# xuyongzhi/Automatic-As-built-Reconstruction

Measured on AMD Instinct MI355X. Metric: scenes/sec (fwd+bwd), higher is better.
Workload: dtype f32

## Files before the change

automatic-as-built-reconstruction_amd/_hip.py:

```python
import ctypes as C
import os

import torch

_HERE = os.path.dirname(os.path.abspath(__file__))
LIB_PATH = os.path.join(_HERE, "lib", "libaabr_hip.so")

_lib = None
META_WORDS = 16
ABI_VERSION = 640

_vp, _i64, _i32, _f32 = C.c_void_p, C.c_int64, C.c_int, C.c_float
_i32p = C.POINTER(C.c_int32)
_f32p = C.POINTER(C.c_float)
_i64p = C.POINTER(C.c_int64)



class AabrRoiLevel(C.Structure):
    _fields_ = [("feats", C.c_void_p), ("cellmap", C.c_void_p), ("height", C.c_int32), ("width", C.c_int32),
                ("zsize", C.c_int32), ("nb", C.c_int32), ("V", C.c_int64), ("row_offset", C.c_int64),
                ("spatial_scale", C.c_float), ("reserved", C.c_int32)]


class AabrRpnMap(C.Structure):
    _fields_ = [("features", C.c_void_p), ("rows", C.c_int64), ("objectness", C.c_void_p),
                ("box_regression", C.c_void_p), ("d_features", C.c_void_p)]


class AabrMlpWindow(C.Structure):
    _fields_ = [("n_rois", C.c_int64), ("ph", C.c_int32), ("pw", C.c_int32), ("R", C.c_int32), ("wlen", C.c_int32),
                ("blocks", C.c_int32), ("w0", C.c_int32 * 2)]


_lvp = C.POINTER(AabrRoiLevel)
_mwp = C.POINTER(AabrMlpWindow)
_rmp = C.POINTER(AabrRpnMap)
_ppv = C.POINTER(C.c_void_p)
_SIGS = {
    "aabr_version": (C.c_int, []),
    "aabr_build_flags": (C.c_int, []),
    "aabr_last_error": (C.c_char_p, []),
    "aabr_set_knob": (C.c_int, [C.c_char_p, C.c_int, C.c_int]),
    "aabr_quantize_points": (C.c_int, [_vp, _i32, _i64, C.c_double, _vp, _vp, _i64, _vp, _vp, _i32, _vp]),
    "aabr_input_layer_status_words": (C.c_int64, [_i64]),
    "aabr_input_layer_sites": (C.c_int, [_vp, _i64, _i32, _vp, _i64, _vp, _vp, _vp, _vp, _vp, _vp, _vp, _vp, _vp, _vp]),
    "aabr_input_layer_pack_bits": (C.c_int, [_i64, _i32p]),
# ... 74 lines not shown
    "aabr_bn_backward_parts": (C.c_int, [_vp, _vp, _vp, _vp, _i64, _i32, _vp, _vp, _vp, _vp, _vp, _vp, _f32, _vp, _i32,
                                         _vp, _vp, _vp]),
    "aabr_bn_forward_parts": (C.c_int, [_vp, _vp, _i64, _i32, _vp, _vp, _vp, _vp, _vp, _vp, _f32, _f32, _f32, _vp,
                                        _i32, _vp, _vp]),
    "aabr_bn_forward_parts_bf16": (C.c_int, [_vp, _vp, _i64, _i32, _vp, _vp, _vp, _vp, _vp, _vp, _f32, _f32, _f32, _vp,
                                             _i32, _vp, _vp]),
    "aabr_mailbox_create": (C.c_int, [_i64, _vp]),
    "aabr_mailbox_destroy": (C.c_int, [_vp]),
    "aabr_mailbox_post": (C.c_int, [_vp, _i64, _vp, C.c_uint32, _vp]),
    "aabr_conv_wpack_floats": (C.c_int64, [_i32, _i32, _i32]),
    "aabr_conv_forward": (C.c_int, [_vp, _i32, _i64, _vp, _i32, _i64, _vp, _i32, _vp, _vp, _i32, _vp, _vp]),
    "aabr_conv_dw_scratch_floats": (C.c_int64, [_i64, _i32, _i32]),
    "aabr_conv_backward_weight": (C.c_int, [_vp, _i32, _vp, _i32, _i64, _vp, _i32, _i64, _vp, _vp, _vp, _vp]),
    "aabr_conv_dw_chunk_pairs": (C.c_int, [_i64, _i32, _i32, _i32]),
    "aabr_conv_dw_vec_operands": (C.c_int, [_i32, _vp, _i32, _vp, _i32, _i64, _i32, _i64]),
    "aabr_conv_pack_weights2": (C.c_int, [_vp, _i32, _i32, _i32, _vp, _vp, _vp]),
    "aabr_conv_pack_weights2_bf16": (C.c_int, [_vp, _i32, _i32, _i32, _vp, _vp, _vp]),
    "aabr_plan_run": (C.c_int, [_vp, _i32, _vp]),
    "aabr_plan_run_tail": (C.c_int, [_vp, _i32, _vp, C.POINTER(C.c_uint64)]),
    "aabr_plan_tail_join": (C.c_int, [C.c_uint64, _vp]),
    "aabr_plan_tail_sync": (C.c_int, [C.c_uint64]),
    "aabr_plan_tail_release": (C.c_int, [C.c_uint64]),
    "aabr_plan_submit": (C.c_int, [_vp, _i32, _vp, _i32]),
    "aabr_plan_drain": (C.c_int, []),
    "aabr_plan_launcher_stats": (None, [_vp, _vp, _vp]),
    "aabr_geom_run": (C.c_int, [_vp, _i32, _vp]),
    "aabr_add": (C.c_int, [_vp, _vp, _vp, _i64, _i32, _vp]),
    "aabr_cast_storage": (C.c_int, [_vp, _vp, _i64, _i32, _vp]),
    "aabr_sum_counts": (C.c_int, [_vp, _vp, _vp, _i32, _vp]),
    "aabr_conv_pack_job_blocks": (C.c_int64, [_i32, _i32, _i32]),
# ... 346 lines not shown
```

automatic-as-built-reconstruction_amd/csrc/common.h:

```cpp
#pragma once
#include <hip/hip_runtime.h>
#include <stdint.h>
#include <stdio.h>
#include <atomic>
#include "../../include/aabr_hip.h"
#include "conv_tiles.h"

namespace aabr {

void set_error(const char *fmt, ...);

typedef float f32x4 __attribute__((ext_vector_type(4)));
typedef unsigned int u32x4 __attribute__((ext_vector_type(4)));
typedef __bf16 bf16x8 __attribute__((ext_vector_type(8)));

#define AABR_KNOB_LIST(X)                                                                                            \
  X(CONV_WLDS) X(CONV_SMALL) X(CONV_NBW) X(CONV_WPB) X(WIDE_ROWS) X(CONV_WIDE) X(WIDE_NBUF) X(CONV_WIDE_BF16)         \
  X(VOXEL_MEAN) X(WIDE_NCB) X(BN_SMALL) X(WIDE_PRIO) X(PLAN_SIDE_BATCH) X(PLAN_SIDE_PRIO) X(SMALL_WPB) X(SMALL_MAX)   \
  X(WIDE_SPLIT) X(SPLIT_TARGET) X(SPLIT_NBUF) X(SPLIT_MIN_ITEMS) X(CONV_NARROW) X(DW_FULL) X(DW_FULL_MIN) X(DW_FULL_WGS) X(DW_VEC) X(SPLIT_ROWS) X(GEOM_JOBS)      \
  X(CONV_SINGLE) X(SINGLE_ROWS) X(SINGLE_CHUNK) X(SINGLE_BWD_STATS) X(PLAN_TAIL)
#define AABR_KNOB_ENUM(n) K_##n,
enum Knob { AABR_KNOB_LIST(AABR_KNOB_ENUM) K_COUNT };
#undef AABR_KNOB_ENUM
int knob(Knob k);

#define AABR_CHECK_ARG_AS(fn, cond, msg)                            \
  do {                                                              \
    if (!(cond)) { aabr::set_error("%s: %s", fn, msg); return AABR_EINVAL; } \
  } while (0)
#define AABR_CHECK_ARG(cond, msg) AABR_CHECK_ARG_AS(__func__, cond, msg)

#define AABR_CHECK_LAUNCH()                                                   \
  do {                                                                        \
    hipError_t e__ = hipGetLastError();                                       \
    if (e__ != hipSuccess) {                                                  \
// ... 110 lines not shown
```

automatic-as-built-reconstruction_amd/csrc/conv_dw.hip:

```cpp
#include "common.h"
#include "conv_dw_tiles.h"
#include "offset_pairs.h"

namespace aabr {

extern thread_local const char *g_last_variant;

__device__ inline float ldf(const float *p, int64_t i) { return p[i]; }
__device__ inline float ldf(const __bf16 *p, int64_t i) { return (float)p[i]; }

typedef float f32x2 __attribute__((ext_vector_type(2)));
template <int N> __device__ inline void ld_row(float (&d)[N], const float *p) {
  if constexpr (N == 4) {
    const f32x4 v = *reinterpret_cast<const f32x4 *>(p);
    d[0] = v[0]; d[1] = v[1]; d[2] = v[2]; d[3] = v[3];
  } else if constexpr (N == 2) {
    const f32x2 v = *reinterpret_cast<const f32x2 *>(p);
    d[0] = v[0]; d[1] = v[1];
  } else d[0] = p[0];
}
template <int N> __device__ inline void ld_row(__bf16 (&)[N], const __bf16 *) {}
template <bool V> struct DwForm { static constexpr bool value = V; };

template <int CB, int NB, typename T>
__global__ __launch_bounds__(256) __attribute__((amdgpu_waves_per_eu(2))) void k_conv_dw_pairs(const T *__restrict__ in, int ci,
                                                       const T *__restrict__ d_out, int co, int64_t V,
                                                       const int32_t *__restrict__ words, int vol,
                                                       int chunk_pairs, float *__restrict__ partial, int form) {
  __shared__ f32x4 red[CB * NB][64];
  constexpr bool kF32 = sizeof(T) == 4;
  const int direct = form & 1;
  const bool vin = kF32 && CB > 1 && (form & (kDwVecIn << 1)), vout = kF32 && NB > 1 && (form & (kDwVecOut << 1));
  const int wave = threadIdx.x >> 6, lane = threadIdx.x & 63;
  const int g = lane >> 4, c16 = lane & 15;
  const int nnb = nnb_of(co);
  const int tiles_n = (nnb + NB - 1) / NB;
  const int tile = blockIdx.y;
  const int cb0 = (tile / tiles_n) * CB, nb0 = (tile % tiles_n) * NB;
  const int chunk = blockIdx.x;
  int k, c0, c1;
  if (!dw_chunk_range(words, vol, chunk_pairs, direct, chunk, lane, k, c0, c1)) return;
  const int rk = words[k];
  const int p0 = c0 + wave * (chunk_pairs / 4);
  int p1 = p0 + chunk_pairs / 4;
  if (p1 > c1) p1 = c1;
  const int2 *pairs = reinterpret_cast<const int2 *>(words + op_hdr(vol) + (int64_t)vol * op_nb256(V)) +
                      (int64_t)k * V;
  f32x4 acc[CB][NB];
#pragma unroll
  for (int a = 0; a < CB; ++a)
#pragma unroll
    for (int b = 0; b < NB; ++b) acc[a][b] = (f32x4){0.f, 0.f, 0.f, 0.f};

  const int cA = ci - 1, nA = co - 1;
// ... 118 lines not shown
    }
  }
#pragma unroll
  for (int a = 0; a < CB; ++a)
#pragma unroll
    for (int b = 0; b < NB; ++b) {
      f32x4 t = red[a * NB + b][lane];
#pragma unroll
      for (int r = 0; r < 4; ++r) {
        int c = cb0 * 16 + dw_tile_row(vin, CB, g, r, a), n = nb0 * 16 + dw_tile_col(vout, NB, c16, b);
        if (c < ci && n < co) P[(int64_t)c * co + n] = t[r];
      }
    }
}

typedef short s16x4 __attribute__((ext_vector_type(4)));

template <int CB, int NB>
__global__ __launch_bounds__(256) void k_conv_dw_pairs_bf16(const __bf16 *__restrict__ in, int ci,
                                                            const __bf16 *__restrict__ d_out, int co, int64_t V,
                                                            const int32_t *__restrict__ words, int vol,
                                                            int chunk_pairs, float *__restrict__ partial, int direct) {
  constexpr int SX = CB * 32 + 16, SG = NB * 32 + 16;
  constexpr int XCH = CB * 2, GCH = NB * 2;
  constexpr int XIT = (32 * XCH) / 64, GIT = (32 * GCH) / 64;
  __shared__ f32x4 red[CB * NB][64];
  __shared__ __attribute__((aligned(16))) unsigned char stage[4][32 * (SX + SG)];
  const int wave = threadIdx.x >> 6, lane = threadIdx.x & 63;
  const int g = lane >> 4, c16 = lane & 15;
  const int nnb = nnb_of(co);
  const int tiles_n = (nnb + NB - 1) / NB;
  const int tile = blockIdx.y;
  const int cb0 = (tile / tiles_n) * CB, nb0 = (tile % tiles_n) * NB;
  const int chunk = blockIdx.x;
  int k, c0, c1;
  if (!dw_chunk_range(words, vol, chunk_pairs, direct, chunk, lane, k, c0, c1)) return;
  const int p0 = c0 + wave * (chunk_pairs / 4);
  int p1 = p0 + chunk_pairs / 4;
  if (p1 > c1) p1 = c1;
  const int2 *pairs = reinterpret_cast<const int2 *>(words + op_hdr(vol) + (int64_t)vol * op_nb256(V)) +
                      (int64_t)k * V;
  unsigned char *xs = stage[wave], *gs = stage[wave] + 32 * SX;
  f32x4 acc[CB][NB];
#pragma unroll
  for (int a = 0; a < CB; ++a)
#pragma unroll
    for (int b = 0; b < NB; ++b) acc[a][b] = (f32x4){0.f, 0.f, 0.f, 0.f};

  u32x4 xr[XIT], gr[GIT];
// ... 75 lines not shown
    __syncthreads();
  }
  if (wave != 0) return;
  float *P = partial + (int64_t)(direct ? k : chunk) * ci * co;
#pragma unroll
  for (int a = 0; a < CB; ++a)
#pragma unroll
    for (int b = 0; b < NB; ++b) {
      f32x4 t = red[a * NB + b][lane];
#pragma unroll
      for (int r = 0; r < 4; ++r) {
        int c = (cb0 + a) * 16 + g * 4 + r, n = (nb0 + b) * 16 + c16;
        if (c < ci && n < co) P[(int64_t)c * co + n] = t[r];
      }
    }
}

constexpr int kDwMinPer = 128;
__device__ inline int64_t dw_range_per(int64_t rtot, int n_wg) {
  const int64_t per = (rtot + n_wg - 1) / n_wg;
  return per < kDwMinPer ? kDwMinPer : per;
}
__device__ inline int wave_incl_scan(int v, int lane) {
#pragma unroll
  for (int d = 1; d < 64; d <<= 1) {
    const int u = __shfl_up(v, d);
    if (lane >= d) v += u;
  }
  return v;
}
// ... 241 lines not shown
    } else if (k >= k0 + 64) ne += (int)__popcll(nz);
    base += __shfl(incl, 63);
  }
  float s = 0.0f;
  if (ck > 0 && i < cico) {
    const int64_t per = dw_range_per(base, n_wg);
    const int64_t w0 = sk / per, w1 = (sk + ck - 1) / per;
#pragma unroll 4
    for (int64_t w = w0 + sl; w <= w1; w += 4) s += partial[(w + ne) * cico + i];
  }
  red[sl][col] = s;
  __syncthreads();
  if (sl == 0 && i < cico) dW[(int64_t)k * cico + i] = (red[0][col] + red[1][col]) + (red[2][col] + red[3][col]);
}

__global__ __launch_bounds__(256) void k_conv_dw_reduce(const float *__restrict__ partial,
                                                        const int32_t *__restrict__ words, int vol,
                                                        int chunk_pairs, int64_t cico, float *__restrict__ dW) {
  __shared__ float red[4][64];
  const int k = blockIdx.y, col = threadIdx.x & 63, sl = threadIdx.x >> 6;
  const int64_t i = (int64_t)blockIdx.x * 64 + col;
  const int32_t *cstart = words + vol + (chunk_pairs == 256 ? vol + 1 : 0);
  const int c0 = cstart[k], c1 = cstart[k + 1];
  float s = 0.0f;
  if (i < cico) {
#pragma unroll 8
    for (int c = c0 + sl; c < c1; c += 4) s += partial[(int64_t)c * cico + i];
  }
  red[sl][col] = s;
  __syncthreads();
  if (sl == 0 && i < cico) dW[(int64_t)k * cico + i] = (red[0][col] + red[1][col]) + (red[2][col] + red[3][col]);
}

template <typename T>
__global__ __launch_bounds__(256) void k_col_sum_partial(const T *__restrict__ x, int64_t rows, int co, int S,
                                                         float *__restrict__ part) {
  __shared__ float red[4][64];
  const int col = blockIdx.x * 64 + (threadIdx.x & 63), sub = threadIdx.x >> 6, sl = blockIdx.y;
  float s = 0.0f;
  if (col < co)
    for (int64_t r = (int64_t)sl * 4 + sub; r < rows; r += (int64_t)S * 4) s += ldf(x, r * co + col);
  red[sub][threadIdx.x & 63] = s;
  __syncthreads();
  if (sub == 0 && col < co)
    part[(int64_t)sl * co + col] = (red[0][threadIdx.x] + red[1][threadIdx.x]) + (red[2][threadIdx.x] + red[3][threadIdx.x]);
}
// ... 41 lines not shown
  static constexpr DwInst<DwFullFn<float>> full[] = {AABR_DW_FULL(f32, false)};
};
template <> struct DwTables<__bf16> {
  static constexpr DwInst<DwPairsFn<__bf16>> pairs[] = {
      AABR_DW_BF16(1, 1), AABR_DW_BF16(1, 2), AABR_DW_BF16(1, 4), AABR_DW_BF16(2, 1), AABR_DW_BF16(2, 2),
      AABR_DW_BF16(2, 4), AABR_DW_BF16(4, 1), AABR_DW_BF16(4, 2), AABR_DW_BF16(4, 4),
      AABR_DW_MFMA(2, 2), AABR_DW_MFMA(2, 4), AABR_DW_MFMA(4, 2), AABR_DW_MFMA(4, 4)};
  static constexpr DwInst<DwFullFn<__bf16>> full[] = {AABR_DW_FULL(bf16, true)};
};
template <typename Fn, size_t N>
static const DwInst<Fn> *dw_inst(const DwInst<Fn> (&tab)[N], const DwKernel &k) {
  for (const DwInst<Fn> &e : tab)
    if (e.k == k) return &e;
  return nullptr;
}

static int dw_pairs_form(const DwLaunch &d, int n_in, int n_out, const void *in_feats, const void *d_out, const float *dst) {
  const int vec = d.k.kind == kDwPairs ? dw_vec_operands(d.k.bf16, n_in, n_out, d.k.cb, d.k.nb, (uintptr_t)in_feats,
                                                          (uintptr_t)d_out, knob(K_DW_VEC)) : 0;
  const int st16 = (vec & kDwVecOut) && d.k.nb == 4 && ((uintptr_t)dst & 15) == 0;
  return d.direct | vec << 1 | st16 << 3;
}

extern "C" int aabr_conv_dw_vec_operands(int bf16, const void *in_feats, int n_in, const void *d_out, int n_out,
                                         int64_t V_out, int vol, int64_t max_chunks) {
  if (n_in <= 0 || n_out <= 0 || vol <= 0 || V_out <= 0 || max_chunks <= 0) return 0;
  const bool bf = bf16 != 0, aligned16 = ((uintptr_t)in_feats & 15) == 0 && ((uintptr_t)d_out & 15) == 0;
  const DwLaunch d = conv_dw_launch(bf, n_in, n_out, V_out, vol, max_chunks, aligned16,
                                    DwKnobs{knob(K_DW_FULL), knob(K_DW_FULL_MIN), knob(K_DW_FULL_WGS)});
  return d.k.kind == kDwPairs ? dw_vec_operands(bf, n_in, n_out, d.k.cb, d.k.nb, (uintptr_t)in_feats, (uintptr_t)d_out,
// ... 54 lines not shown
extern "C" int aabr_conv_backward_weight(const float *in_feats, int n_in, const float *d_out, int n_out,
                                         int64_t V_out, const int32_t *pairs, int vol, int64_t max_chunks,
                                         float *dW, float *d_bias, float *scratch, void *stream_) {
  return conv_backward_weight_t<float>(in_feats, n_in, d_out, n_out, V_out, pairs, vol, max_chunks, dW, d_bias,
                                       scratch, stream_);
}

extern "C" int aabr_conv_backward_weight_bf16(const uint16_t *in_feats, int n_in, const uint16_t *d_out,
                                              int n_out, int64_t V_out, const int32_t *pairs, int vol,
                                              int64_t max_chunks, float *dW, float *d_bias, float *scratch,
                                              void *stream_) {
  return conv_backward_weight_t<__bf16>(reinterpret_cast<const __bf16 *>(in_feats), n_in,
                                        reinterpret_cast<const __bf16 *>(d_out), n_out, V_out, pairs, vol,
                                        max_chunks, dW, d_bias, scratch, stream_);
}
```

automatic-as-built-reconstruction_amd/csrc/conv_dw_tiles.h:

```cpp
#pragma once
#include <stdint.h>
#include "conv_tiles.h"

namespace aabr {

AABR_HD int dw_chunk(int64_t V, int vol, int n_in, int n_out) {
  return ((int64_t)vol * V <= (1ll << 21) && (int64_t)n_in * n_out <= 64 * 64) ? 256 : 1024;
}

struct DwKnobs { int full, full_min, full_wgs; };

enum DwKind { kDwPairs, kDwPairsMfma, kDwFull };
enum DwReduce { kDwReduceNone, kDwReduceChunks, kDwReduceRanges };

struct DwKernel {
  int kind;
  bool bf16;
  int cb, nb;
};
inline bool operator==(const DwKernel &a, const DwKernel &b) {
  return a.kind == b.kind && a.bf16 == b.bf16 && a.cb == b.cb && a.nb == b.nb;
}
struct DwLaunch {
  DwKernel k;
// ... 56 lines not shown
  if (d.n_wg) {
    d.k = {kDwFull, bf16, 0, 0};
    d.grid_x = d.n_wg;
    d.grid_y = (n_in >> 7) * (n_out >> 7);
    d.reduce = kDwReduceRanges;
    return d;
  }
  d.k.kind = dw_mfma16(bf16, n_in, n_out, aligned16) && d.k.cb > 1 && d.k.nb > 1 ? kDwPairsMfma : kDwPairs;
  d.k.bf16 = bf16;
  d.grid_x = d.direct ? vol : max_chunks;
  d.grid_y = d.tiles;
  d.reduce = d.direct ? kDwReduceNone : kDwReduceChunks;
  return d;
}

}
```

automatic-as-built-reconstruction_amd/csrc/plan.hip:

```cpp
#include "common.h"
#include "plan_records.h"
#include "plan_tail.h"
#include <string.h>
#include <chrono>
#include <condition_variable>
#include <deque>
#include <mutex>
#include <string>
#include <thread>
#include <vector>

namespace aabr {

typedef __bf16 bf16x4 __attribute__((ext_vector_type(4)));

template <typename T>
__global__ __launch_bounds__(256) void k_add2(const T *__restrict__ a, const T *__restrict__ b, T *__restrict__ o,
                                              int64_t n) {
  const int64_t i = ((int64_t)blockIdx.x * 256 + threadIdx.x) * 4;
  if (i + 3 < n) {
    if constexpr (sizeof(T) == 4) {
      const float4 x = *reinterpret_cast<const float4 *>(a + i), y = *reinterpret_cast<const float4 *>(b + i);
      *reinterpret_cast<float4 *>(o + i) = make_float4(x.x + y.x, x.y + y.y, x.z + y.z, x.w + y.w);
    } else {
// ... 154 lines not shown
  hipStream_t own = nullptr;
  size_t pending = 0;
  std::vector<hipEvent_t> events;
  hipEvent_t get(size_t k) {
    while (events.size() <= k) {
      hipEvent_t e = nullptr;
      if (hipEventCreateWithFlags(&e, hipEventDisableTiming) != hipSuccess) return nullptr;
      events.push_back(e);
    }
    return events[k];
  }
};
thread_local SideStream g_side;

constexpr int kPlanTailDefault = 2;
struct DevStreams { hipStream_t tail = nullptr, shared = nullptr; };
std::mutex g_dev_mu;
std::vector<DevStreams> g_dev_streams;
TailTickets g_tickets;

inline int plan_tail_mode() {
  const int v = knob(K_PLAN_TAIL);
  return (v == 0 || v == 1 || v == 2) ? v : kPlanTailDefault;
}

int dev_stream(bool shared, hipStream_t *out) {
  int dev = 0;
  AABR_CHECK_HIP(hipGetDevice(&dev));
  std::lock_guard<std::mutex> l(g_dev_mu);
  if ((int)g_dev_streams.size() <= dev) g_dev_streams.resize(dev + 1);
// ... 197 lines not shown
  if (batch < 1 || batch > 64) batch = 1;
  std::vector<int> deferred;
  auto fail = [&](int rc) {
    if (n_pending) hipStreamSynchronize(g_side.stream);
    if (n_tail) hipStreamSynchronize(tail_stream);
    return rc;
  };
  auto join_side = [&]() -> int {
    hipEvent_t e = g_side.get(n_events++);
    if (e == nullptr) { aabr::set_error("aabr_plan_run: event creation failed"); return AABR_ELAUNCH; }
    hipError_t he = hipEventRecord(e, g_side.stream);
    if (he == hipSuccess) he = hipStreamWaitEvent(main_stream, e, 0);
    if (he != hipSuccess) { aabr::set_error("aabr_plan_run: HIP error %s", hipGetErrorString(he)); return AABR_ELAUNCH; }
    return AABR_OK;
  };
  auto flush = [&]() -> int {
    if (deferred.empty()) return AABR_OK;
    if (!g_side.stream && tail_mode == 2) {
      const int rc = dev_stream(true, &g_side.stream);
      if (rc != AABR_OK) return rc;
    }
    if (!g_side.stream) {
      int lo = 0, hi = 0;
      const int v = knob(K_PLAN_SIDE_PRIO);
      if ((v == 1 || v == 2) && hipDeviceGetStreamPriorityRange(&lo, &hi) == hipSuccess)
        AABR_CHECK_HIP(hipStreamCreateWithPriority(&g_side.stream, hipStreamNonBlocking, v == 1 ? lo : hi));
      else
        AABR_CHECK_HIP(hipStreamCreateWithFlags(&g_side.stream, hipStreamNonBlocking));
      g_side.own = g_side.stream;
    }
    hipEvent_t e = g_side.get(n_events++);
    AABR_CHECK_ARG(e != nullptr, "event creation failed");
    AABR_CHECK_HIP(hipEventRecord(e, main_stream));
    AABR_CHECK_HIP(hipStreamWaitEvent(g_side.stream, e, 0));
    for (int idx : deferred) {
      ++n_pending;
      const int rc = plan_dispatch(ops[idx], (void *)g_side.stream);
      if (rc != AABR_OK) { deferred.clear(); return rc; }
    }
    deferred.clear();
    return AABR_OK;
  };
  auto fork_tail = [&]() -> int {
    if (!tail_stream) {
      const int rc = dev_stream(tail_mode == 2, &tail_stream);
      if (rc != AABR_OK) return rc;
    }
    hipEvent_t e = g_side.get(n_events++);
    AABR_CHECK_ARG(e != nullptr, "event creation failed");
// ... 26 lines not shown
      rc = plan_dispatch(o, (void *)tail_stream);
      if (rc != AABR_OK) return fail(rc);
      continue;
    }
    in_tail_run = false;
    if (o.flags & AABR_PLAN_JOIN) {
      const int rc = flush();
      if (rc != AABR_OK) return fail(rc);
      if (n_pending) {
        const int jr = join_side();
        if (jr != AABR_OK) return fail(jr);
        n_pending = 0;
      }
    }
    if (o.flags & AABR_PLAN_SIDE) {
      deferred.push_back(j);
      if ((int)deferred.size() >= batch) {
        const int rc = flush();
        if (rc != AABR_OK) return fail(rc);
      }
      continue;
    }
    if (o.kind == AABR_PLAN_CAST) {
      const size_t es_in = (o.flags & AABR_PLAN_TO_BF16) ? 4 : 2, es_out = (o.flags & AABR_PLAN_TO_BF16) ? 2 : 4;
      auto overlaps = [](const void *a, size_t na, const void *b, size_t nb) {
        const uintptr_t a0 = (uintptr_t)a, b0 = (uintptr_t)b;
        return a0 < b0 + nb && b0 < a0 + na;
      };
      int m = 1;
      while (j + m < n_ops && m < kCastJobsMax && ops[j + m].kind == AABR_PLAN_CAST &&
// ... 329 lines not shown
```

automatic-as-built-reconstruction_amd/sparseconvnet/planExecutor.py:

```python
import ctypes
import functools
import threading

import torch
from torch.autograd import Function

import _hip
from _hip import stream, check
from . import SCN
from . import plan_records as R
from .plan_records import (K_CONV, K_WIDE, K_DW, K_BNF, K_BNB, K_ADD, K_CAST, K_WSPLIT, K_NARROW, K_SINGLE,
                           K_TAIL_JOIN, F_BF16, F_TO_BF16, F_SIDE, F_JOIN, F_TAIL)
from .sparseConvNetTensor import SparseConvNetTensor
from .sequential import Sequential
from .tables import AddTable, ConcatTable
from .identity import Identity
from .batchNormalization import BatchNormalization
from .submanifoldConvolution import SubmanifoldConvolution
from .convolution import Convolution
from .deconvolution import Deconvolution
from .fullConvolution import FullConvolution

_ALIGN = 256
BF16 = torch.bfloat16
# ... 703 lines not shown
        self._tmp = []
        gouts = [g.contiguous() if g is not None else None for g in gouts]
        bw = t.backward(tuple(g is not None for g in gouts), need_dx)
        gbufs, bops = bw["gbufs"], bw["ops"]
        offs, total = _offsets(gbufs, V)
        garena = torch.empty(max(total, 1), dtype=torch.uint8, device=self.dev)
        hooked = grad_segments > 1 and on_grads_ready is not None
        gparams = (torch.zeros if hooked else torch.empty)(max(bw["ptotal"], 1), dtype=torch.float32, device=self.dev)
        gbase, pbase, sbase = garena.data_ptr(), gparams.data_ptr(), self.stat.data_ptr()
        AD = (A, [gbase + o for o in offs], [_dp(g) for g in gouts])
        for (b, _), g in zip(t.outs, gouts):
            if g is not None:
                lvl, planes, dt = t.fbufs[b]
                assert g.dtype == dt and g.numel() == V[lvl] * planes
        books = self.books
        dws, dwmc = 0, []
        for op in bops:
            if op[0] == "dw":
                mc = books[op[6]][op[7]].max_chunks(op[4], op[5])
                dwmc.append(mc)
                dws = max(dws, mc * op[4] * op[5])
        dwmc.reverse()
        dwws = _hip.workspace("dw", dws, torch.float32, self.dev).data_ptr() if dws else 0
        bnws = _hip.workspace("bn", t.bn_floats, torch.float32, self.dev).data_ptr() if t.bn_floats else 0
        SZ, off = R.SIZE, 0
        buf = bytearray((len(bops) * 2 + 1) * SZ)
        (flag_patch, flag_at), (bn_patch, bn_at) = R.CONV_BWD_STATS
        dw_side = F_SIDE if dw_side_stream else 0
        nseg = grad_segments if (grad_segments > 1 and on_grads_ready is not None) else 1
        cut = [(len(bops) * (q + 1)) // nseg for q in range(nseg)] if nseg > 1 else []
        inv = sorted((o, i) for i, o in bw["poff"].items()) if nseg > 1 else []
        done_floats, seg_no, next_inv = 0, 0, 0
        claimed = bw.get("claimed")
        if claimed is None:
            claimed = bw["claimed"] = set()
            for i, op in enumerate(bops):
                if op[0] == "din":
# ... 49 lines not shown
                                                   V[lvl], n_out, g, p_w, pt, flags, 0,
                                                   AD[res[0]][res[1]] if res is not None else 0)
                    if nparts:
                        last_din = (gx, off0, nparts, n_out)
                else:
                    off, _ = self.conv_launch(self.route(n_in, n_out, V[lo], V[lvl], g.vol, bf), buf, off,
                                              AD[gy[0]][gy[1]], V[lo], n_in, AD[tmp[0]][tmp[1]], V[lvl], n_out, g, p_w,
                                              pt, flags)
                    R.ADD.pack_into(buf, off, K_ADD, flg, V[lvl] * n_out, AD[res[0]][res[1]], AD[tmp[0]][tmp[1]],
                                    AD[gx[0]][gx[1]])
                    off += SZ
            elif kind == "dw":
                _, x, gy, lo, n_in, n_out, book, side, pg, flg = op
                g = books[book][side]
                R.CONV_DW.pack_into(buf, off, K_DW, flg | dw_side, n_in, n_out, g.vol, V[lo], dwmc.pop(), A[x],
                                    AD[gy[0]][gy[1]], g.pairs().data_ptr(), pbase + pg, 0, dwws)
                off += SZ
            elif kind == "bn":
                _, x, gx, y, gy, lvl, planes, flg, leak, st, p_w, pw, pb, p_b, res = op
                if V[lvl]:
                    parts, nparts, ld = 0, 0, last_din
                    if (conv_bn_bwd_stats and ld is not None and ld[0] == gy and ld[3] == planes
                            and (flg == F_BF16 or (not flg and leak >= 0.0))):
                        nparts = ld[2]
                        if bstat is None:
                            bstat = _hip.workspace("conv_bwd_stats", (max(V) // 64 + 1) * 2 * t.max_planes,
                                                   torch.float64, self.dev).data_ptr()
                        parts = bstat
                        flag_patch.pack_into(buf, ld[1] + flag_at, 1, leak)
                        bn_patch.pack_into(buf, ld[1] + bn_at, bstat, A[x], sbase + st * 4,
                                           A[y] if flg == F_BF16 else sbase + (st + planes) * 4, p_w, p_b)
# ... 161 lines not shown
```

include/aabr_hip.h:

```cpp
#ifndef AABR_HIP_H
#define AABR_HIP_H
#include <stdint.h>
#ifdef __cplusplus
extern "C" {
#endif

#define AABR_OK 0
#define AABR_EINVAL (-1)
#define AABR_ELAUNCH (-2)
#define AABR_ERANGE (-3)

const char *aabr_last_error(void);
#define AABR_ABI_VERSION 640
int aabr_version(void);
int aabr_set_knob(const char *name, int value, int unset);
int aabr_build_flags(void);
#define AABR_META_WORDS 16

int aabr_quantize_points(const void *xyz, int is_double, int64_t n, double scale, const void *xyz_min,
                         const int32_t *full_scale_dev, int64_t batch_index, int64_t *locs,
                         float *feats_xyz, int feat_stride, void *stream);


int64_t aabr_input_layer_status_words(int64_t n);
// ... 158 lines not shown
                      int64_t V_out, const int32_t *blocks, int vol, const float *W,
                      const float *bias, int flags, float *wpack, void *stream);
int aabr_conv_pack_weights2(const float *W, int vol, int n_in, int n_out, float *wpack_fwd,
                            float *wpack_t, void *stream);
int aabr_conv_pack_weights2_bf16(const float *W, int vol, int n_in, int n_out, uint16_t *wpack_fwd,
                                 uint16_t *wpack_t, void *stream);
int64_t aabr_conv_pack_job_blocks(int vol, int n_in, int n_out);
int aabr_conv_pack_weights_jobs(const void *jobs_dev, int n_jobs, int64_t total_blocks, void *stream);
int64_t aabr_conv_dw_scratch_floats(int64_t max_chunks, int n_in, int n_out);
int aabr_conv_dw_chunk_pairs(int64_t V_out, int vol, int n_in, int n_out);
int aabr_conv_dw_vec_operands(int bf16, const void *in_feats, int n_in, const void *d_out, int n_out, int64_t V_out,
                              int vol, int64_t max_chunks);
int aabr_conv_backward_weight(const float *in_feats, int n_in, const float *d_out, int n_out,
                              int64_t V_out, const int32_t *pairs, int vol, int64_t max_chunks,
                              float *dW, float *d_bias, float *scratch, void *stream);

int64_t aabr_bn_scratch_floats(int planes);
int aabr_bn_forward(const float *in, float *out, int64_t rows, int planes, float *save_mean,
                    float *save_invstd, float *running_mean, float *running_var,
                    const float *weight, const float *bias, float eps, float momentum,
                    int train, float leakiness, float *scratch, void *stream);
int aabr_bn_backward(const float *in, float *d_in, const float *out, const float *d_out,
                     int64_t rows, int planes, const float *save_mean, const float *save_invstd,
                     const float *weight, const float *bias, float *d_weight, float *d_bias, float leakiness,
                     float *scratch, void *stream);

int aabr_bn_backward_add(const float *in, float *d_in, const float *out, const float *d_out, int64_t rows,
                         int planes, const float *save_mean, const float *save_invstd, const float *weight,
                         const float *bias, float *d_weight, float *d_bias, float leakiness, float *scratch,
                         const float *d_in_add, void *stream);
// ... 423 lines not shown
```

Before: 356.1.

## Batch small weight-gradient convolutions into grouped multi-job kernel launches

Adds grouped kernels that run several small sparse-conv weight-gradient jobs, plus their chunk reductions, in a single launch, picking the job by a block-index lookup in a job table passed as a kernel argument. The plan executor collects consecutive side-stream weight-gradient ops that fit a group and dispatches them together, and the Python side lays out separate scratch offsets so grouped jobs do not overlap. The aim is to cut launch count and per-launch overhead for many tiny backward-weight kernels. The cost is a linear job search per block, a larger kernel argument, more scratch memory, and grouping that only applies when all jobs share one kernel instance.

```diff
diff --git a/automatic-as-built-reconstruction_amd/_hip.py b/automatic-as-built-reconstruction_amd/_hip.py
--- a/automatic-as-built-reconstruction_amd/_hip.py
+++ b/automatic-as-built-reconstruction_amd/_hip.py
@@ -31,6 +31,12 @@
 class AabrMlpWindow(C.Structure):
     _fields_ = [("n_rois", C.c_int64), ("ph", C.c_int32), ("pw", C.c_int32), ("R", C.c_int32), ("wlen", C.c_int32),
                 ("blocks", C.c_int32), ("w0", C.c_int32 * 2)]
+
+
+class AabrDwJob(C.Structure):
+    _fields_ = [("in_feats", C.c_void_p), ("d_out", C.c_void_p), ("pairs", C.c_void_p), ("dW", C.c_void_p),
+                ("scratch", C.c_void_p), ("V_out", C.c_int64), ("max_chunks", C.c_int64), ("n_in", C.c_int32),
+                ("n_out", C.c_int32), ("vol", C.c_int32), ("reserved", C.c_int32)]
 
 
 _lvp = C.POINTER(AabrRoiLevel)
@@ -135,6 +141,12 @@
     "aabr_conv_backward_weight": (C.c_int, [_vp, _i32, _vp, _i32, _i64, _vp, _i32, _i64, _vp, _vp, _vp, _vp]),
     "aabr_conv_dw_chunk_pairs": (C.c_int, [_i64, _i32, _i32, _i32]),
     "aabr_conv_dw_vec_operands": (C.c_int, [_i32, _vp, _i32, _vp, _i32, _i64, _i32, _i64]),
+    "aabr_conv_backward_weight_group": (C.c_int, [C.POINTER(AabrDwJob), _i32, _vp]),
+    "aabr_conv_backward_weight_group_bf16": (C.c_int, [C.POINTER(AabrDwJob), _i32, _vp]),
+    "aabr_conv_dw_group_place": (C.c_int64, [_i32, _i32, _i32, _i64, _i32, _i64, _i32, _i64p, C.POINTER(C.c_int), _i64p]),
+    "aabr_conv_dw_group_small": (C.c_int, [_i32, _vp, _i32, _vp, _i32, _i64, _i32, _i64, _i32]),
+    "aabr_conv_dw_group_counts": (None, [_i64p]),
+    "aabr_conv_dw_group_limits": (C.c_int, [_i64p]),
     "aabr_conv_pack_weights2": (C.c_int, [_vp, _i32, _i32, _i32, _vp, _vp, _vp]),
     "aabr_conv_pack_weights2_bf16": (C.c_int, [_vp, _i32, _i32, _i32, _vp, _vp, _vp]),
     "aabr_plan_run": (C.c_int, [_vp, _i32, _vp]),
diff --git a/automatic-as-built-reconstruction_amd/csrc/common.h b/automatic-as-built-reconstruction_amd/csrc/common.h
--- a/automatic-as-built-reconstruction_amd/csrc/common.h
+++ b/automatic-as-built-reconstruction_amd/csrc/common.h
@@ -18,7 +18,7 @@
   X(CONV_WLDS) X(CONV_SMALL) X(CONV_NBW) X(CONV_WPB) X(WIDE_ROWS) X(CONV_WIDE) X(WIDE_NBUF) X(CONV_WIDE_BF16)         \
   X(VOXEL_MEAN) X(WIDE_NCB) X(BN_SMALL) X(WIDE_PRIO) X(PLAN_SIDE_BATCH) X(PLAN_SIDE_PRIO) X(SMALL_WPB) X(SMALL_MAX)   \
   X(WIDE_SPLIT) X(SPLIT_TARGET) X(SPLIT_NBUF) X(SPLIT_MIN_ITEMS) X(CONV_NARROW) X(DW_FULL) X(DW_FULL_MIN) X(DW_FULL_WGS) X(DW_VEC) X(SPLIT_ROWS) X(GEOM_JOBS)      \
-  X(CONV_SINGLE) X(SINGLE_ROWS) X(SINGLE_CHUNK) X(SINGLE_BWD_STATS) X(PLAN_TAIL)
+  X(CONV_SINGLE) X(SINGLE_ROWS) X(SINGLE_CHUNK) X(SINGLE_BWD_STATS) X(PLAN_TAIL) X(PLAN_DW_GROUP)
 #define AABR_KNOB_ENUM(n) K_##n,
 enum Knob { AABR_KNOB_LIST(AABR_KNOB_ENUM) K_COUNT };
 #undef AABR_KNOB_ENUM
diff --git a/automatic-as-built-reconstruction_amd/csrc/conv_dw.hip b/automatic-as-built-reconstruction_amd/csrc/conv_dw.hip
--- a/automatic-as-built-reconstruction_amd/csrc/conv_dw.hip
+++ b/automatic-as-built-reconstruction_amd/csrc/conv_dw.hip
@@ -23,10 +23,9 @@
 template <bool V> struct DwForm { static constexpr bool value = V; };
 
 template <int CB, int NB, typename T>
-__global__ __launch_bounds__(256) __attribute__((amdgpu_waves_per_eu(2))) void k_conv_dw_pairs(const T *__restrict__ in, int ci,
-                                                       const T *__restrict__ d_out, int co, int64_t V,
-                                                       const int32_t *__restrict__ words, int vol,
-                                                       int chunk_pairs, float *__restrict__ partial, int form) {
+__device__ __forceinline__ void dw_pairs_body(const T *__restrict__ in, int ci, const T *__restrict__ d_out, int co, int64_t V,
+                                              const int32_t *__restrict__ words, int vol, int chunk_pairs,
+                                              float *__restrict__ partial, int form, const int chunk, const int tile) {
   __shared__ f32x4 red[CB * NB][64];
   constexpr bool kF32 = sizeof(T) == 4;
   const int direct = form & 1;
@@ -35,9 +34,7 @@
   const int g = lane >> 4, c16 = lane & 15;
   const int nnb = nnb_of(co);
   const int tiles_n = (nnb + NB - 1) / NB;
-  const int tile = blockIdx.y;
   const int cb0 = (tile / tiles_n) * CB, nb0 = (tile % tiles_n) * NB;
-  const int chunk = blockIdx.x;
   int k, c0, c1;
   if (!dw_chunk_range(words, vol, chunk_pairs, direct, chunk, lane, k, c0, c1)) return;
   const int rk = words[k];
@@ -186,13 +183,21 @@
     }
 }
 
+template <int CB, int NB, typename T>
+__global__ __launch_bounds__(256) __attribute__((amdgpu_waves_per_eu(2))) void k_conv_dw_pairs(const T *__restrict__ in, int ci,
+                                                       const T *__restrict__ d_out, int co, int64_t V,
+                                                       const int32_t *__restrict__ words, int vol,
+                                                       int chunk_pairs, float *__restrict__ partial, int form) {
+  dw_pairs_body<CB, NB, T>(in, ci, d_out, co, V, words, vol, chunk_pairs, partial, form, blockIdx.x, blockIdx.y);
+}
+
 typedef short s16x4 __attribute__((ext_vector_type(4)));
 
 template <int CB, int NB>
-__global__ __launch_bounds__(256) void k_conv_dw_pairs_bf16(const __bf16 *__restrict__ in, int ci,
-                                                            const __bf16 *__restrict__ d_out, int co, int64_t V,
-                                                            const int32_t *__restrict__ words, int vol,
-                                                            int chunk_pairs, float *__restrict__ partial, int direct) {
+__device__ __forceinline__ void dw_pairs_bf16_body(const __bf16 *__restrict__ in, int ci, const __bf16 *__restrict__ d_out,
+                                                   int co, int64_t V, const int32_t *__restrict__ words, int vol,
+                                                   int chunk_pairs, float *__restrict__ partial, int direct, const int chunk,
+                                                   const int tile) {
   constexpr int SX = CB * 32 + 16, SG = NB * 32 + 16;
   constexpr int XCH = CB * 2, GCH = NB * 2;
   constexpr int XIT = (32 * XCH) / 64, GIT = (32 * GCH) / 64;
@@ -202,9 +207,7 @@
   const int g = lane >> 4, c16 = lane & 15;
   const int nnb = nnb_of(co);
   const int tiles_n = (nnb + NB - 1) / NB;
-  const int tile = blockIdx.y;
   const int cb0 = (tile / tiles_n) * CB, nb0 = (tile % tiles_n) * NB;
-  const int chunk = blockIdx.x;
   int k, c0, c1;
   if (!dw_chunk_range(words, vol, chunk_pairs, direct, chunk, lane, k, c0, c1)) return;
   const int p0 = c0 + wave * (chunk_pairs / 4);
@@ -310,6 +313,49 @@
         if (c < ci && n < co) P[(int64_t)c * co + n] = t[r];
       }
     }
+}
+
+template <int CB, int NB>
+__global__ __launch_bounds__(256) void k_conv_dw_pairs_bf16(const __bf16 *__restrict__ in, int ci,
+                                                            const __bf16 *__restrict__ d_out, int co, int64_t V,
+                                                            const int32_t *__restrict__ words, int vol,
+                                                            int chunk_pairs, float *__restrict__ partial, int direct) {
+  dw_pairs_bf16_body<CB, NB>(in, ci, d_out, co, V, words, vol, chunk_pairs, partial, direct, blockIdx.x, blockIdx.y);
+}
+
+struct DwJobDev {
+  const void *in, *d_out;
+  const int32_t *words;
+  float *dst;
+  int64_t V;
+  int32_t ci, co, vol, chunk_pairs, form, gx;
+};
+struct DwJobs {
+  DwJobDev j[kDwGroupMaxJobs];
+  uint32_t first[kDwGroupMaxJobs + 1];
+  int n;
+};
+static_assert(sizeof(DwJobs) <= 3072, "the job table is a kernel argument");
+__device__ inline int dw_job_of(const uint32_t *first, int n, unsigned b) {
+  int j = 0;
+  while (j + 1 < n && b >= first[j + 1]) ++j;
+  return j;
+}
+template <int CB, int NB, typename T>
+__global__ __launch_bounds__(256) __attribute__((amdgpu_waves_per_eu(2))) void k_conv_dw_pairs_jobs(const DwJobs js) {
+  const int j = dw_job_of(js.first, js.n, blockIdx.x);
+  const DwJobDev &J = js.j[j];
+  const unsigned l = blockIdx.x - js.first[j];
+  dw_pairs_body<CB, NB, T>((const T *)J.in, J.ci, (const T *)J.d_out, J.co, J.V, J.words, J.vol, J.chunk_pairs, J.dst, J.form,
+                           (int)(l % (unsigned)J.gx), (int)(l / (unsigned)J.gx));
+}
+template <int CB, int NB>
+__global__ __launch_bounds__(256) void k_conv_dw_pairs_bf16_jobs(const DwJobs js) {
+  const int j = dw_job_of(js.first, js.n, blockIdx.x);
+  const DwJobDev &J = js.j[j];
+  const unsigned l = blockIdx.x - js.first[j];
+  dw_pairs_bf16_body<CB, NB>((const __bf16 *)J.in, J.ci, (const __bf16 *)J.d_out, J.co, J.V, J.words, J.vol, J.chunk_pairs,
+                             J.dst, J.form & 1, (int)(l % (unsigned)J.gx), (int)(l / (unsigned)J.gx));
 }
 
 constexpr int kDwMinPer = 128;
@@ -581,12 +627,12 @@
   if (sl == 0 && i < cico) dW[(int64_t)k * cico + i] = (red[0][col] + red[1][col]) + (red[2][col] + red[3][col]);
 }
 
-__global__ __launch_bounds__(256) void k_conv_dw_reduce(const float *__restrict__ partial,
-                                                        const int32_t *__restrict__ words, int vol,
-                                                        int chunk_pairs, int64_t cico, float *__restrict__ dW) {
+__device__ __forceinline__ void dw_reduce_body(const float *__restrict__ partial, const int32_t *__restrict__ words, int vol,
+                                               int chunk_pairs, int64_t cico, float *__restrict__ dW, const int bx,
+                                               const int k) {
   __shared__ float red[4][64];
-  const int k = blockIdx.y, col = threadIdx.x & 63, sl = threadIdx.x >> 6;
-  const int64_t i = (int64_t)blockIdx.x * 64 + col;
+  const int col = threadIdx.x & 63, sl = threadIdx.x >> 6;
+  const int64_t i = (int64_t)bx * 64 + col;
   const int32_t *cstart = words + vol + (chunk_pairs == 256 ? vol + 1 : 0);
   const int c0 = cstart[k], c1 = cstart[k + 1];
   float s = 0.0f;
@@ -597,6 +643,29 @@
   red[sl][col] = s;
   __syncthreads();
   if (sl == 0 && i < cico) dW[(int64_t)k * cico + i] = (red[0][col] + red[1][col]) + (red[2][col] + red[3][col]);
+}
+__global__ __launch_bounds__(256) void k_conv_dw_reduce(const float *__restrict__ partial,
+                                                        const int32_t *__restrict__ words, int vol,
+                                                        int chunk_pairs, int64_t cico, float *__restrict__ dW) {
+  dw_reduce_body(partial, words, vol, chunk_pairs, cico, dW, blockIdx.x, blockIdx.y);
+}
+struct DwReduceJobDev {
+  const float *partial;
+  const int32_t *words;
+  float *dW;
+  int64_t cico;
+  int32_t vol, chunk_pairs, nbx, pad;
+};
+struct DwReduceJobs {
+  DwReduceJobDev j[kDwGroupMaxJobs];
+  uint32_t first[kDwGroupMaxJobs + 1];
+  int n;
+};
+__global__ __launch_bounds__(256) void k_conv_dw_reduce_jobs(const DwReduceJobs js) {
+  const int j = dw_job_of(js.first, js.n, blockIdx.x);
+  const DwReduceJobDev &J = js.j[j];
+  const unsigned l = blockIdx.x - js.first[j];
+  dw_reduce_body(J.partial, J.words, J.vol, J.chunk_pairs, J.cico, J.dW, (int)(l % (unsigned)J.nbx), (int)(l / (unsigned)J.nbx));
 }
 
 template <typename T>
@@ -668,6 +737,25 @@
     if (e.k == k) return &e;
   return nullptr;
 }
+using DwJobsFn = void (*)(const DwJobs);
+template <typename T> struct DwJobTables;
+#define AABR_DWJ_F32(CB, NB) \
+  {{kDwPairs, false, CB, NB}, "k_conv_dw_pairs_jobs<" #CB "," #NB ",float>", k_conv_dw_pairs_jobs<CB, NB, float>}
+#define AABR_DWJ_BF16(CB, NB) \
+  {{kDwPairs, true, CB, NB}, "k_conv_dw_pairs_jobs<" #CB "," #NB ",bf16>", k_conv_dw_pairs_jobs<CB, NB, __bf16>}
+#define AABR_DWJ_MFMA(CB, NB) \
+  {{kDwPairsMfma, true, CB, NB}, "k_conv_dw_pairs_bf16_jobs<" #CB "," #NB ">", k_conv_dw_pairs_bf16_jobs<CB, NB>}
+template <> struct DwJobTables<float> {
+  static constexpr DwInst<DwJobsFn> pairs[] = {
+      AABR_DWJ_F32(1, 1), AABR_DWJ_F32(1, 2), AABR_DWJ_F32(1, 4), AABR_DWJ_F32(2, 1), AABR_DWJ_F32(2, 2),
+      AABR_DWJ_F32(2, 4), AABR_DWJ_F32(4, 1), AABR_DWJ_F32(4, 2), AABR_DWJ_F32(4, 4)};
+};
+template <> struct DwJobTables<__bf16> {
+  static constexpr DwInst<DwJobsFn> pairs[] = {
+      AABR_DWJ_BF16(1, 1), AABR_DWJ_BF16(1, 2), AABR_DWJ_BF16(1, 4), AABR_DWJ_BF16(2, 1), AABR_DWJ_BF16(2, 2),
+      AABR_DWJ_BF16(2, 4), AABR_DWJ_BF16(4, 1), AABR_DWJ_BF16(4, 2), AABR_DWJ_BF16(4, 4),
+      AABR_DWJ_MFMA(2, 2), AABR_DWJ_MFMA(2, 4), AABR_DWJ_MFMA(4, 2), AABR_DWJ_MFMA(4, 4)};
+};
 
 static int dw_pairs_form(const DwLaunch &d, int n_in, int n_out, const void *in_feats, const void *d_out, const float *dst) {
   const int vec = d.k.kind == kDwPairs ? dw_vec_operands(d.k.bf16, n_in, n_out, d.k.cb, d.k.nb, (uintptr_t)in_feats,
@@ -752,3 +840,91 @@
                                         reinterpret_cast<const __bf16 *>(d_out), n_out, V_out, pairs, vol,
                                         max_chunks, dW, d_bias, scratch, stream_);
 }
+
+static std::atomic<long long> g_dw_group_launches{0}, g_dw_group_jobs{0}, g_dw_group_reduces{0};
+
+extern "C" void aabr_conv_dw_group_counts(int64_t *out3) {
+  out3[0] = g_dw_group_launches.load();
+  out3[1] = g_dw_group_jobs.load();
+  out3[2] = g_dw_group_reduces.load();
+}
+
+extern "C" int aabr_conv_dw_group_limits(int64_t *out5) {
+  out5[0] = kDwGroupMaxJobs; out5[1] = kDwGroupMaxWgs; out5[2] = kDwGroupMaxGroupWgs; out5[3] = kDwGroupMaxScratchFloats;
+  out5[4] = kDwGroupScratchAlign;
+  return AABR_OK;
+}
+
+extern "C" int aabr_conv_dw_group_small(int bf16, const void *in_feats, int n_in, const void *d_out, int n_out, int64_t V_out,
+                                        int vol, int64_t max_chunks, int has_bias) {
+  const bool aligned16 = ((uintptr_t)in_feats & 15) == 0 && ((uintptr_t)d_out & 15) == 0;
+  const DwGroupRec r{bf16 != 0, n_in, n_out, vol, V_out, max_chunks, aligned16, has_bias != 0, 0};
+  DwLaunch d{};
+  return dw_group_small(r, DwKnobs{knob(K_DW_FULL), knob(K_DW_FULL_MIN), knob(K_DW_FULL_WGS)}, d) ? (int)(d.grid_x * d.grid_y) : 0;
+}
+
+extern "C" int64_t aabr_conv_dw_group_place(int bf16, int n_in, int n_out, int64_t V_out, int vol, int64_t max_chunks,
+                                            int has_bias, int64_t *cursor, int *count, int64_t *need_out) {
+  const DwGroupRec r{bf16 != 0, n_in, n_out, vol, V_out, max_chunks, true, has_bias != 0, 0};
+  DwLaunch d{};
+  const bool small = dw_group_small(r, DwKnobs{knob(K_DW_FULL), knob(K_DW_FULL_MIN), knob(K_DW_FULL_WGS)}, d);
+  const int64_t need = small ? dw_group_need(d, n_in, n_out) : max_chunks * n_in * n_out;
+  if (need_out) *need_out = need;
+  return dw_group_place(small, need, *cursor, *count);
+}
+
+template <typename T>
+static int conv_backward_weight_group_t(const AabrDwJob *jobs, int n_jobs, void *stream_) {
+  hipStream_t st = (hipStream_t)stream_;
+  AABR_CHECK_ARG(jobs && n_jobs >= 1 && n_jobs <= kDwGroupMaxJobs, "bad job count");
+  const bool bf = sizeof(T) == 2;
+  const DwKnobs kn{knob(K_DW_FULL), knob(K_DW_FULL_MIN), knob(K_DW_FULL_WGS)};
+  DwJobs pj{};
+  DwReduceJobs rj{};
+  DwGroup g;
+  uint64_t wgs = 0, rwgs = 0;
+  for (int i = 0; i < n_jobs; ++i) {
+    const AabrDwJob &a = jobs[i];
+    AABR_CHECK_ARG(a.in_feats && a.d_out && a.pairs && a.dW, "null pointer");
+    const bool aligned16 = ((uintptr_t)a.in_feats & 15) == 0 && ((uintptr_t)a.d_out & 15) == 0;
+    const DwGroupRec r{bf, a.n_in, a.n_out, a.vol, a.V_out, a.max_chunks, aligned16, false, (uint64_t)(uintptr_t)a.scratch};
+    DwLaunch d{};
+    AABR_CHECK_ARG(dw_group_small(r, kn, d), "a job is not a small weight gradient");
+    AABR_CHECK_ARG(!dw_mfma16(bf, a.n_in, a.n_out, aligned16) || (a.n_in <= 4096 && a.n_out <= 4096), "bad sizes");
+    AABR_CHECK_ARG(d.direct || a.scratch, "null scratch");
+    AABR_CHECK_ARG(dw_group_fits(g, r, d), "the jobs are not one group (instance, caps or overlapping partial regions)");
+    dw_group_add(g, r, d);
+    float *dst = d.to_scratch ? a.scratch : a.dW;
+    pj.j[i] = DwJobDev{a.in_feats, a.d_out, a.pairs, dst, a.V_out, a.n_in, a.n_out, a.vol, d.chunk_pairs,
+                       dw_pairs_form(d, a.n_in, a.n_out, a.in_feats, a.d_out, dst), (int32_t)d.grid_x};
+    pj.first[i] = (uint32_t)wgs;
+    wgs += (uint64_t)(d.grid_x * d.grid_y);
+    if (d.reduce == kDwReduceChunks) {
+      const int64_t cico = (int64_t)a.n_in * a.n_out, nbx = ceil_div(cico, 64);
+      rj.j[rj.n] = DwReduceJobDev{a.scratch, a.pairs, a.dW, cico, a.vol, d.chunk_pairs, (int32_t)nbx, 0};
+      rj.first[rj.n++] = (uint32_t)rwgs;
+      rwgs += (uint64_t)(nbx * a.vol);
+    }
+  }
+  AABR_CHECK_ARG(rwgs < (1ull << 31), "too many reduce workgroups");
+  pj.n = n_jobs;
+  pj.first[n_jobs] = (uint32_t)wgs;
+  rj.first[rj.n] = (uint32_t)rwgs;
+  const auto *e = dw_inst(DwJobTables<T>::pairs, g.k);
+  AABR_CHECK_ARG(e, "no kernel instance for this launch");
+  g_last_variant = e->name;
+  hipLaunchKernelGGL(e->fn, dim3((unsigned)wgs), dim3(256), 0, st, pj);
+  if (rj.n) hipLaunchKernelGGL(k_conv_dw_reduce_jobs, dim3((unsigned)rwgs), dim3(256), 0, st, rj);
+  AABR_CHECK_LAUNCH();
+  g_dw_group_launches.fetch_add(1);
+  g_dw_group_jobs.fetch_add(n_jobs);
+  if (rj.n) g_dw_group_reduces.fetch_add(1);
+  return AABR_OK;
+}
+
+extern "C" int aabr_conv_backward_weight_group(const AabrDwJob *jobs, int n_jobs, void *stream) {
+  return conv_backward_weight_group_t<float>(jobs, n_jobs, stream);
+}
+extern "C" int aabr_conv_backward_weight_group_bf16(const AabrDwJob *jobs, int n_jobs, void *stream) {
+  return conv_backward_weight_group_t<__bf16>(jobs, n_jobs, stream);
+}
diff --git a/automatic-as-built-reconstruction_amd/csrc/conv_dw_tiles.h b/automatic-as-built-reconstruction_amd/csrc/conv_dw_tiles.h
--- a/automatic-as-built-reconstruction_amd/csrc/conv_dw_tiles.h
+++ b/automatic-as-built-reconstruction_amd/csrc/conv_dw_tiles.h
@@ -94,4 +94,82 @@
   return d;
 }
 
+constexpr int kDwGroupMaxJobs = 32;
+constexpr int kDwGroupMaxWgs = 1024;
+constexpr int64_t kDwGroupMaxGroupWgs = 16384;
+constexpr int64_t kDwGroupMaxScratchFloats = 16ll << 20;
+constexpr int64_t kDwGroupScratchAlign = 64;
+
+struct DwGroupRec {
+  bool bf16;
+  int n_in, n_out, vol;
+  int64_t V_out, max_chunks;
+  bool aligned16, has_bias;
+  uint64_t scratch;
+};
+inline int64_t dw_group_need(const DwLaunch &d, int n_in, int n_out) {
+  return d.to_scratch ? d.grid_x * n_in * n_out : 0;
 }
+inline bool dw_group_small(const DwGroupRec &r, const DwKnobs &kn, DwLaunch &d) {
+  if (r.n_in <= 0 || r.n_out <= 0 || r.vol <= 0 || r.vol > 65535 || r.V_out <= 0 || r.max_chunks <= 0 || r.has_bias)
+    return false;
+  d = conv_dw_launch(r.bf16, r.n_in, r.n_out, r.V_out, r.vol, r.max_chunks, r.aligned16, kn);
+  return d.k.kind != kDwFull && d.tiles <= 65535 && d.grid_x * d.grid_y <= kDwGroupMaxWgs;
+}
+struct DwGroup {
+  int n = 0;
+  DwKernel k{};
+  int64_t wgs = 0, floats = 0;
+  uint64_t lo[kDwGroupMaxJobs], hi[kDwGroupMaxJobs];
+  void clear() { n = 0; wgs = 0; floats = 0; }
+};
+inline bool dw_group_fits(const DwGroup &g, const DwGroupRec &r, const DwLaunch &d) {
+  if (g.n == 0) return true;
+  const int64_t need = dw_group_need(d, r.n_in, r.n_out);
+  if (g.n >= kDwGroupMaxJobs || !(g.k == d.k) || g.wgs + d.grid_x * d.grid_y > kDwGroupMaxGroupWgs ||
+      g.floats + need > kDwGroupMaxScratchFloats)
+    return false;
+  const uint64_t lo = r.scratch, hi = r.scratch + (uint64_t)need * 4;
+  for (int i = 0; i < g.n; ++i)
+    if (lo < g.hi[i] && g.lo[i] < hi) return false;
+  return true;
+}
+inline void dw_group_add(DwGroup &g, const DwGroupRec &r, const DwLaunch &d) {
+  const int64_t need = dw_group_need(d, r.n_in, r.n_out);
+  if (g.n == 0) g.k = d.k;
+  g.lo[g.n] = r.scratch;
+  g.hi[g.n] = r.scratch + (uint64_t)need * 4;
+  ++g.n;
+  g.wgs += d.grid_x * d.grid_y;
+  g.floats += need;
+}
+inline int dw_group_scan(const DwGroupRec *r, const unsigned char *part_end, int n, const DwKnobs &kn, int *group) {
+  DwGroup g;
+  int n_groups = 0;
+  for (int i = 0; i < n; ++i) {
+    DwLaunch d{};
+    if (!dw_group_small(r[i], kn, d)) {
+      if (g.n) { ++n_groups; g.clear(); }
+      group[i] = -1;
+    } else {
+      if (!dw_group_fits(g, r[i], d)) { ++n_groups; g.clear(); }
+      dw_group_add(g, r[i], d);
+      group[i] = n_groups;
+    }
+    if (part_end && part_end[i] && g.n) { ++n_groups; g.clear(); }
+  }
+  if (g.n) ++n_groups;
+  return n_groups;
+}
+
+inline int64_t dw_group_place(bool small, int64_t need, int64_t &cursor, int &count) {
+  if (!small) { cursor = 0; count = 0; return 0; }
+  const int64_t al = (need + kDwGroupScratchAlign - 1) / kDwGroupScratchAlign * kDwGroupScratchAlign;
+  if (count >= kDwGroupMaxJobs || cursor + al > kDwGroupMaxScratchFloats) { cursor = 0; count = 0; }
+  const int64_t off = cursor;
+  cursor += al;
+  ++count;
+  return off;
+}
+
+}
diff --git a/automatic-as-built-reconstruction_amd/csrc/plan.hip b/automatic-as-built-reconstruction_amd/csrc/plan.hip
--- a/automatic-as-built-reconstruction_amd/csrc/plan.hip
+++ b/automatic-as-built-reconstruction_amd/csrc/plan.hip
@@ -1,4 +1,5 @@
 #include "common.h"
+#include "conv_dw_tiles.h"
 #include "plan_records.h"
 #include "plan_tail.h"
 #include <string.h>
@@ -192,6 +193,7 @@
 thread_local SideStream g_side;
 
 constexpr int kPlanTailDefault = 2;
+constexpr int kPlanDwGroupDefault = 1;
 struct DevStreams { hipStream_t tail = nullptr, shared = nullptr; };
 std::mutex g_dev_mu;
 std::vector<DevStreams> g_dev_streams;
@@ -419,8 +421,7 @@
     if (he != hipSuccess) { aabr::set_error("aabr_plan_run: HIP error %s", hipGetErrorString(he)); return AABR_ELAUNCH; }
     return AABR_OK;
   };
-  auto flush = [&]() -> int {
-    if (deferred.empty()) return AABR_OK;
+  auto side_stream = [&]() -> int {
     if (!g_side.stream && tail_mode == 2) {
       const int rc = dev_stream(true, &g_side.stream);
       if (rc != AABR_OK) return rc;
@@ -434,10 +435,72 @@
         AABR_CHECK_HIP(hipStreamCreateWithFlags(&g_side.stream, hipStreamNonBlocking));
       g_side.own = g_side.stream;
     }
+    return AABR_OK;
+  };
+  auto fork_side = [&]() -> int {
+    const int rc = side_stream();
+    if (rc != AABR_OK) return rc;
     hipEvent_t e = g_side.get(n_events++);
     AABR_CHECK_ARG(e != nullptr, "event creation failed");
     AABR_CHECK_HIP(hipEventRecord(e, main_stream));
     AABR_CHECK_HIP(hipStreamWaitEvent(g_side.stream, e, 0));
+    return AABR_OK;
+  };
+  const bool dw_grouping = knob(K_PLAN_DW_GROUP) == kKnobUnset ? kPlanDwGroupDefault != 0 : knob(K_PLAN_DW_GROUP) != 0;
+  const DwKnobs dw_knobs{knob(K_DW_FULL), knob(K_DW_FULL_MIN), knob(K_DW_FULL_WGS)};
+  DwGroup dw_group;
+  std::vector<int> dw_members;
+  auto close_group = [&]() -> int {
+    if (dw_members.empty()) return AABR_OK;
+    int rc = fork_side();
+    if (rc == AABR_OK) {
+      n_pending += dw_members.size();
+      if (dw_members.size() == 1) rc = plan_dispatch(ops[dw_members[0]], (void *)g_side.stream);
+      else {
+        AabrDwJob jobs[kDwGroupMaxJobs];
+        for (size_t i = 0; i < dw_members.size(); ++i) {
+          const PlanConvDw r{ops[dw_members[i]]};
+          jobs[i] = AabrDwJob{r.in(), r.d_out(), idx(r.pairs()), f32(r.dW()), f32(r.scratch()), r.V_out(), r.max_chunks(),
+                              r.n_in(), r.n_out(), r.vol(), 0};
+        }
+        const bool bf = (ops[dw_members[0]].flags & AABR_PLAN_BF16) != 0;
+        rc = bf ? aabr_conv_backward_weight_group_bf16(jobs, (int)dw_members.size(), (void *)g_side.stream)
+                : aabr_conv_backward_weight_group(jobs, (int)dw_members.size(), (void *)g_side.stream);
+      }
+    }
+    dw_members.clear();
+    dw_group.clear();
+    return rc;
+  };
+  auto collect_dw = [&](int j, int &rc) -> bool {
+    rc = AABR_OK;
+    const AabrPlanOp &o = ops[j];
+    if (!dw_grouping || o.kind != AABR_PLAN_CONV_DW) return false;
+    const PlanConvDw r{o};
+    const bool aligned16 = ((uintptr_t)r.in() & 15) == 0 && ((uintptr_t)r.d_out() & 15) == 0;
+    const DwGroupRec g{(o.flags & AABR_PLAN_BF16) != 0, r.n_in(), r.n_out(), r.vol(), r.V_out(), r.max_chunks(), aligned16,
+                       r.d_bias() != nullptr, (uint64_t)(uintptr_t)r.scratch()};
+    DwLaunch d{};
+    if (!r.in() || !r.d_out() || !r.pairs() || !r.dW() || !dw_group_small(g, dw_knobs, d) || (d.to_scratch && !r.scratch()))
+      return false;
+    if (!dw_group_fits(dw_group, g, d)) {
+      rc = close_group();
+      if (rc != AABR_OK) return true;
+    }
+    dw_group_add(dw_group, g, d);
+    dw_members.push_back(j);
+    return true;
+  };
+  auto flush = [&]() -> int {
+    {
+      const int rc = close_group();
+      if (rc != AABR_OK) { deferred.clear(); return rc; }
+    }
+    if (deferred.empty()) return AABR_OK;
+    {
+      const int rc = fork_side();
+      if (rc != AABR_OK) return rc;
+    }
     for (int idx : deferred) {
       ++n_pending;
       const int rc = plan_dispatch(ops[idx], (void *)g_side.stream);
@@ -494,6 +557,16 @@
       }
     }
     if (o.flags & AABR_PLAN_SIDE) {
+      if (deferred.empty()) {
+        int rc = AABR_OK;
+        const bool taken = collect_dw(j, rc);
+        if (rc != AABR_OK) return fail(rc);
+        if (taken) continue;
+      }
+      if (!dw_members.empty()) {
+        const int rc = close_group();
+        if (rc != AABR_OK) return fail(rc);
+      }
       deferred.push_back(j);
       if ((int)deferred.size() >= batch) {
         const int rc = flush();
diff --git a/automatic-as-built-reconstruction_amd/sparseconvnet/planExecutor.py b/automatic-as-built-reconstruction_amd/sparseconvnet/planExecutor.py
--- a/automatic-as-built-reconstruction_amd/sparseconvnet/planExecutor.py
+++ b/automatic-as-built-reconstruction_amd/sparseconvnet/planExecutor.py
@@ -741,13 +741,19 @@
                 lvl, planes, dt = t.fbufs[b]
                 assert g.dtype == dt and g.numel() == V[lvl] * planes
         books = self.books
-        dws, dwmc = 0, []
+        dws, dwmc, dwoff = 0, [], []
+        cur, cnt, need = ctypes.c_int64(0), ctypes.c_int(0), ctypes.c_int64(0)
         for op in bops:
             if op[0] == "dw":
-                mc = books[op[6]][op[7]].max_chunks(op[4], op[5])
+                g = books[op[6]][op[7]]
+                mc = g.max_chunks(op[4], op[5])
                 dwmc.append(mc)
-                dws = max(dws, mc * op[4] * op[5])
+                o = int(self.lib.aabr_conv_dw_group_place(1 if op[9] == F_BF16 else 0, op[4], op[5], V[op[3]], g.vol, mc, 0,
+                                                          ctypes.byref(cur), ctypes.byref(cnt), ctypes.byref(need)))
+                dwoff.append(o * 4)
+                dws = max(dws, mc * op[4] * op[5], o + need.value)
         dwmc.reverse()
+        dwoff.reverse()
         dwws = _hip.workspace("dw", dws, torch.float32, self.dev).data_ptr() if dws else 0
         bnws = _hip.workspace("bn", t.bn_floats, torch.float32, self.dev).data_ptr() if t.bn_floats else 0
         SZ, off = R.SIZE, 0
@@ -827,7 +833,7 @@
                 _, x, gy, lo, n_in, n_out, book, side, pg, flg = op
                 g = books[book][side]
                 R.CONV_DW.pack_into(buf, off, K_DW, flg | dw_side, n_in, n_out, g.vol, V[lo], dwmc.pop(), A[x],
-                                    AD[gy[0]][gy[1]], g.pairs().data_ptr(), pbase + pg, 0, dwws)
+                                    AD[gy[0]][gy[1]], g.pairs().data_ptr(), pbase + pg, 0, dwws + dwoff.pop())
                 off += SZ
             elif kind == "bn":
                 _, x, gx, y, gy, lvl, planes, flg, leak, st, p_w, pw, pb, p_b, res = op
diff --git a/include/aabr_hip.h b/include/aabr_hip.h
--- a/include/aabr_hip.h
+++ b/include/aabr_hip.h
@@ -196,6 +196,21 @@
 int aabr_conv_backward_weight(const float *in_feats, int n_in, const float *d_out, int n_out,
                               int64_t V_out, const int32_t *pairs, int vol, int64_t max_chunks,
                               float *dW, float *d_bias, float *scratch, void *stream);
+typedef struct AabrDwJob {
+  const void *in_feats, *d_out;
+  const int32_t *pairs;
+  float *dW, *scratch;
+  int64_t V_out, max_chunks;
+  int32_t n_in, n_out, vol, reserved;
+} AabrDwJob;
+int aabr_conv_backward_weight_group(const AabrDwJob *jobs, int n_jobs, void *stream);
+int aabr_conv_backward_weight_group_bf16(const AabrDwJob *jobs, int n_jobs, void *stream);
+int64_t aabr_conv_dw_group_place(int bf16, int n_in, int n_out, int64_t V_out, int vol, int64_t max_chunks, int has_bias,
+                                 int64_t *cursor, int *count, int64_t *need_out);
+int aabr_conv_dw_group_small(int bf16, const void *in_feats, int n_in, const void *d_out, int n_out, int64_t V_out, int vol,
+                             int64_t max_chunks, int has_bias);
+void aabr_conv_dw_group_counts(int64_t *out3);
+int aabr_conv_dw_group_limits(int64_t *out5);
 
 int64_t aabr_bn_scratch_floats(int planes);
 int aabr_bn_forward(const float *in, float *out, int64_t rows, int planes, float *save_mean,
```

Result: no change. 358.5 (median of 6 runs) (+0.7%).
